# audio-visual/Audio_Visual_Deepfake_Detection

Measured on NVIDIA B200. Metric: videos/sec localization inference (fwd+decode+soft-NMS), higher is better.
Workload: dtype bf16

## Files before the change

audio_visual_deepfake_detection_b200/csrc/mlp_fused.cu:

```cuda
#include <cuda.h>
#include <stdlib.h>
#include <string.h>
#include "../../include/avdf.h"
#include "tc_ptx.cuh"

namespace avdf {
namespace mlpf {
using namespace tc;

constexpr int C = 256, HID = 1024, BM = 128, HC = 128, NCHUNK = HID / HC;
constexpr int UNIT = 128 * 64 * 2;
constexpr int RING = 5;
#ifndef AVDF_MLP_GELU_WARPS
#define AVDF_MLP_GELU_WARPS 8
#endif
constexpr int EPI_WARPS = 8;
constexpr int GELU_WARPS = AVDF_MLP_GELU_WARPS;
static_assert(GELU_WARPS == 8 || GELU_WARPS == 16, "GELU warps");
constexpr int GCOLS = HC / (GELU_WARPS / 4);
constexpr int THREADS = 128 + GELU_WARPS * 32;
constexpr int OFF_X = 0;
constexpr int OFF_H = OFF_X + 4 * UNIT;
constexpr int OFF_STG = OFF_H + 2 * UNIT;
constexpr int OFF_RING = OFF_STG + EPI_WARPS * 4096;
constexpr int OFF_VEC = OFF_RING + RING * UNIT;
constexpr int OFF_PART = OFF_VEC + (HID + 6 * C) * 4;
constexpr int OFF_BAR = OFF_PART + 2 * BM * 8;
constexpr int SMEM_BYTES = OFF_BAR + 512 + 1024;

struct Params {
  CUtensorMap x_map, w1_map, w2_map;
  CUtensorMap res_map, out_map;
  CUtensorMap att_map, wo_map, skip_map;
  const float* bo; const float* gamma_a; const float* ln2_w; const float* ln2_b;
  int y_store;
  void* out_h;
  const float* b1; const float* b2; const float* gamma; const unsigned char* row_mask;
  int rows, tiles;
  int oh_t, oh_pitch, oh_row0;
  unsigned idesc, idesc2;
  unsigned long long* dbg;
};
__device__ __forceinline__ unsigned long long gtime_ns() { unsigned long long t; asm volatile("mov.u64 %0, %globaltimer;" : "=l"(t)); return t; }
#define MLPF_TS(role, slot) do { if (p.dbg && blockIdx.x == 0 && it == 0 && (slot) < 96 && (threadIdx.x & 31) == 0) p.dbg[(role) * 96 + (slot)] = gtime_ns(); } while (0)

enum { B_XFULL = 0, B_XEMPTY, B_RFULL, B_REMPTY = B_RFULL + RING, B_A1FULL = B_REMPTY + RING, B_A1EMPTY = B_A1FULL + 2,
       B_HFULL = B_A1EMPTY + 2, B_HEMPTY, B_A2FULL, B_A2EMPTY, B_ATTFULL, B_ATTEMPTY, B_RES, B_RES2 = B_RES + 2 * EPI_WARPS,
       B_COUNT = B_RES2 + 2 * EPI_WARPS };
static_assert(B_COUNT * 8 + 8 <= 512, "barrier block");

template <bool F16, bool PROJ>
__global__ void __launch_bounds__(THREADS, 1) mlp_fused_kernel(const __grid_constant__ Params p) {
  extern __shared__ unsigned char smem_dyn[];
  unsigned char* smem = smem_dyn + ((1024u - (smem_u32(smem_dyn) & 1023u)) & 1023u);
  unsigned char* sx = smem + OFF_X;
  unsigned char* sh = smem + OFF_H;
  unsigned char* sstg = smem + OFF_STG;
  unsigned char* sring = smem + OFF_RING;
  float* s_b1 = reinterpret_cast<float*>(smem + OFF_VEC);
  float* s_b2 = s_b1 + HID;
  float* s_gam = s_b2 + C;
  float* s_bo = s_gam + C; float* s_gama = s_bo + C; float* s_l2w = s_gama + C; float* s_l2b = s_l2w + C;
  float2* s_part = reinterpret_cast<float2*>(smem + OFF_PART);
  uint64_t* bars = reinterpret_cast<uint64_t*>(smem + OFF_BAR);
  uint32_t* tmem_ptr_smem = reinterpret_cast<uint32_t*>(bars + B_COUNT);
  const uint32_t bar_base = smem_u32(bars);
  auto bar = [&](int i) { return bar_base + 8u * (uint32_t)i; };
  const int warp = threadIdx.x >> 5, lane = threadIdx.x & 31;
  const uint32_t rank = cluster_ctarank();
  const int unit0 = (int)(blockIdx.x >> 1), unit_step = (int)(gridDim.x >> 1), n_units = (p.tiles + 1) / 2;
  auto lbar = [&](int i) { return mapa_rank(bar(i), 0u); };
  auto chunk_of = [&](int j) { return j; };

  if (warp == 0 && lane == 0) {
    asm volatile("prefetch.tensormap [%0];" ::"l"(&p.x_map) : "memory");
    asm volatile("prefetch.tensormap [%0];" ::"l"(&p.w1_map) : "memory");
    asm volatile("prefetch.tensormap [%0];" ::"l"(&p.w2_map) : "memory");
    asm volatile("prefetch.tensormap [%0];" ::"l"(&p.res_map) : "memory");
    asm volatile("prefetch.tensormap [%0];" ::"l"(&p.out_map) : "memory");
    if (PROJ) {
      asm volatile("prefetch.tensormap [%0];" ::"l"(&p.att_map) : "memory");
      asm volatile("prefetch.tensormap [%0];" ::"l"(&p.wo_map) : "memory");
      asm volatile("prefetch.tensormap [%0];" ::"l"(&p.skip_map) : "memory");
    }
  }
  if (warp == 1 && lane == 0) {
    mbar_init(bar(B_XFULL), PROJ ? 2 * EPI_WARPS : 1); mbar_init(bar(B_XEMPTY), 1);
    mbar_init(bar(B_ATTFULL), 1); mbar_init(bar(B_ATTEMPTY), EPI_WARPS);
    for (int s = 0; s < RING; ++s) { mbar_init(bar(B_RFULL + s), 1); mbar_init(bar(B_REMPTY + s), 1); }
    for (int s = 0; s < 2; ++s) { mbar_init(bar(B_A1FULL + s), 1); mbar_init(bar(B_A1EMPTY + s), 2 * GELU_WARPS); }
    mbar_init(bar(B_HFULL), 2 * GELU_WARPS); mbar_init(bar(B_HEMPTY), 1);
    mbar_init(bar(B_A2FULL), 1); mbar_init(bar(B_A2EMPTY), 2 * EPI_WARPS);
    for (int s = 0; s < 4 * EPI_WARPS; ++s) mbar_init(bar(B_RES + s), 1);
    asm volatile("fence.mbarrier_init.release.cluster;" ::: "memory");
  }
  if (warp == 2) {
    asm volatile("tcgen05.alloc.cta_group::2.sync.aligned.shared::cta.b32 [%0], %1;" ::"r"(smem_u32(tmem_ptr_smem)), "r"(512u) : "memory");
    asm volatile("tcgen05.relinquish_alloc_permit.cta_group::2.sync.aligned;" ::: "memory");
  }
  if (warp >= 4) {
    for (int i = threadIdx.x - 128; i < HID; i += GELU_WARPS * 32) s_b1[i] = p.b1 ? __ldg(p.b1 + i) : 0.f;
    for (int i = threadIdx.x - 128; i < C; i += GELU_WARPS * 32) {
      s_b2[i] = p.b2 ? __ldg(p.b2 + i) : 0.f;
      s_gam[i] = p.gamma ? __ldg(p.gamma + i) : 1.f;
      if (PROJ) {
        s_bo[i] = p.bo ? __ldg(p.bo + i) : 0.f;
        s_gama[i] = p.gamma_a ? __ldg(p.gamma_a + i) : 1.f;
        s_l2w[i] = __ldg(p.ln2_w + i); s_l2b[i] = __ldg(p.ln2_b + i);
      }
    }
  }
  tcgen05_fence_before();
  cluster_sync_all();
  tcgen05_fence_after();
  const uint32_t tmem_base = *tmem_ptr_smem;
  const uint32_t tm_acc2 = tmem_base + 256u;
  pdl_trigger();
  pdl_wait();

  if (warp == 0) {
    const bool leader = elect_one();
    int stage = 0; uint32_t phase = 0; int it = 0;
    int nu = 0;
    auto begin_slot = [&]() -> uint32_t {
      mbar_wait(bar(B_REMPTY + stage), phase ^ 1);
      MLPF_TS(0, 1 + nu); ++nu;
      if (leader && rank == 0) mbar_arrive_expect_tx(bar(B_RFULL + stage), 2 * UNIT);
      return lbar(B_RFULL + stage);
    };
    auto end_slot = [&]() { __syncwarp(); if (++stage == RING) { stage = 0; phase ^= 1; } };
    auto load_w1 = [&](int chunk, int u) {
      const uint32_t fb = begin_slot();
      if (leader) {
        tma_load_2d_pair(smem_u32(sring + stage * UNIT), &p.w1_map, fb, (2 * u) * 64, chunk * HC + (int)rank * 64);
        tma_load_2d_pair(smem_u32(sring + stage * UNIT + UNIT / 2), &p.w1_map, fb, (2 * u + 1) * 64, chunk * HC + (int)rank * 64);
      }
      end_slot();
    };
    auto load_w2 = [&](int chunk, int sl) {
      const uint32_t fb = begin_slot();
      if (leader) tma_load_2d_pair(smem_u32(sring + stage * UNIT), &p.w2_map, fb, chunk * HC + sl * 64, (int)rank * 128);
      end_slot();
    };
    for (int unit = unit0; unit < n_units; unit += unit_step, ++it) {
      const int tile = 2 * unit + (int)rank;
      nu = 0;
      if (!PROJ) {
        mbar_wait(bar(B_XEMPTY), (uint32_t)(it & 1) ^ 1);
        MLPF_TS(0, 0);
        if (leader) {
          if (rank == 0) mbar_arrive_expect_tx(bar(B_XFULL), 8 * UNIT);
          const uint32_t xb = lbar(B_XFULL);
          for (int s = 0; s < 4; ++s) tma_load_2d_pair(smem_u32(sx + s * UNIT), &p.x_map, xb, s * 64, tile * BM);
        }
        __syncwarp();
      } else {
        mbar_wait(bar(B_ATTEMPTY), (uint32_t)(it & 1) ^ 1);
        MLPF_TS(0, 0);
        if (leader) {
          if (rank == 0) mbar_arrive_expect_tx(bar(B_ATTFULL), 8 * UNIT);
          const uint32_t ab = lbar(B_ATTFULL);
          for (int s = 0; s < 4; ++s) tma_load_2d_pair(smem_u32(sh + s * UNIT), &p.att_map, ab, s * 64, tile * BM);
        }
        __syncwarp();
        for (int sl = 0; sl < 4; ++sl) {
          const uint32_t fb = begin_slot();
          if (leader) tma_load_2d_pair(smem_u32(sring + stage * UNIT), &p.wo_map, fb, sl * 64, (int)rank * 128);
          end_slot();
        }
      }
      for (int u = 0; u < 2; ++u) load_w1(chunk_of(0), u);
      for (int j = 0; j < NCHUNK; ++j) {
        if (j + 1 < NCHUNK)
          for (int u = 0; u < 2; ++u) load_w1(chunk_of(j + 1), u);
        for (int sl = 0; sl < 2; ++sl) load_w2(chunk_of(j), sl);
      }
    }
  } else if (warp == 1 && rank == 0) {
    const bool leader = elect_one();
    int stage = 0; uint32_t phase = 0; int it = 0;
    uint32_t n_a1[2] = {0, 0}, n_h = 0, n_a2e = 0;
    auto g1 = [&](int j) {
      const int b = j & 1;
      mbar_wait(bar(B_A1EMPTY + b), (n_a1[b] & 1) ^ 1);
      tcgen05_fence_after();
      for (int u = 0; u < 2; ++u) {
        mbar_wait(bar(B_RFULL + stage), phase);
        tcgen05_fence_after();
        if (leader) {
#pragma unroll
          for (int ks = 0; ks < 2; ++ks) {
            const uint64_t da = make_sw128_desc(smem_u32(sx + (2 * u + ks) * UNIT));
            const uint64_t db = make_sw128_desc(smem_u32(sring + stage * UNIT + ks * (UNIT / 2)));
#pragma unroll
            for (int k = 0; k < 4; ++k)
              umma_bf16_pair(tmem_base + (uint32_t)(b * HC), da + (uint64_t)(2 * k), db + (uint64_t)(2 * k), p.idesc, (u > 0 || ks > 0 || k > 0) ? 1u : 0u);
          }
          umma_commit_pair(bar(B_REMPTY + stage));
          if (u == 1) umma_commit_pair(bar(B_A1FULL + b));
        }
        __syncwarp();
        if (++stage == RING) { stage = 0; phase ^= 1; }
      }
      ++n_a1[b];
    };
    for (int unit = unit0; unit < n_units; unit += unit_step, ++it) {
      if (PROJ) {
        mbar_wait(bar(B_A2EMPTY), (n_a2e & 1) ^ 1); ++n_a2e;
        mbar_wait(bar(B_ATTFULL), (uint32_t)(it & 1));
        tcgen05_fence_after();
        for (int sl = 0; sl < 4; ++sl) {
          mbar_wait(bar(B_RFULL + stage), phase);
          tcgen05_fence_after();
          if (leader) {
            const uint64_t da = make_sw128_desc(smem_u32(sh + sl * UNIT));
            const uint64_t db = make_sw128_desc(smem_u32(sring + stage * UNIT));
#pragma unroll
            for (int k = 0; k < 4; ++k)
              umma_bf16_pair(tm_acc2, da + (uint64_t)(2 * k), db + (uint64_t)(2 * k), p.idesc2, (sl > 0 || k > 0) ? 1u : 0u);
            umma_commit_pair(bar(B_REMPTY + stage));
            if (sl == 3) umma_commit_pair(bar(B_A2FULL));
          }
          __syncwarp();
          if (++stage == RING) { stage = 0; phase ^= 1; }
        }
      }
      mbar_wait(bar(B_XFULL), (uint32_t)(it & 1));
      tcgen05_fence_after();
      MLPF_TS(1, 0);
      g1(0);
      MLPF_TS(1, 1);
      for (int j = 0; j < NCHUNK; ++j) {
        if (j + 1 < NCHUNK) g1(j + 1);
        MLPF_TS(1, 2 + 4 * j);
        if (j == NCHUNK - 2 && leader) umma_commit_pair(bar(B_XEMPTY));
        if (j == 0) { mbar_wait(bar(B_A2EMPTY), (n_a2e & 1) ^ 1); ++n_a2e; tcgen05_fence_after(); }
        mbar_wait(bar(B_HFULL), n_h & 1);
        tcgen05_fence_after();
        MLPF_TS(1, 3 + 4 * j);
        for (int sl = 0; sl < 2; ++sl) {
          mbar_wait(bar(B_RFULL + stage), phase);
          tcgen05_fence_after();
          if (leader) {
            const uint64_t da = make_sw128_desc(smem_u32(sh + sl * UNIT));
            const uint64_t db = make_sw128_desc(smem_u32(sring + stage * UNIT));
#pragma unroll
            for (int k = 0; k < 4; ++k)
              umma_bf16_pair(tm_acc2, da + (uint64_t)(2 * k), db + (uint64_t)(2 * k), p.idesc2, (PROJ || j > 0 || sl > 0 || k > 0) ? 1u : 0u);
            umma_commit_pair(bar(B_REMPTY + stage));
          }
          __syncwarp();
          if (++stage == RING) { stage = 0; phase ^= 1; }
        }
        if (leader) {
          umma_commit_pair(bar(B_HEMPTY));
          if (j == NCHUNK - 1) umma_commit_pair(bar(B_A2FULL));
        }
        __syncwarp();
        ++n_h;
        MLPF_TS(1, 4 + 4 * j);
      }
    }
  } else if (warp >= 4) {
    const int wi = warp - 4;
    const int q = warp & 3;
    const int cg = wi >> 2;
    const int g = cg & 1;
    const bool fin = wi < EPI_WARPS;
    const int r = q * 32 + lane;
    const int sw7 = lane & 7;
    unsigned char* tA = sstg + (wi & 7) * 4096;
    unsigned char* tB = sh + (wi & 7) * 4096;
    const uint32_t res_bar[2] = {bar(B_RES + 2 * (wi & 7)), bar(B_RES + 2 * (wi & 7) + 1)};
    uint32_t res_phase[2] = {0, 0};
    const uint32_t a1empty_bar[2] = {lbar(B_A1EMPTY), lbar(B_A1EMPTY + 1)};
    const uint32_t hfull_bar = lbar(B_HFULL), a2empty_bar = lbar(B_A2EMPTY);
    uint32_t n_a1[2] = {0, 0}, n_h = 0, n_a2f = 0;
    const uint32_t xfull_bar = lbar(B_XFULL);
    int it = 0;
    for (int unit = unit0; unit < n_units; unit += unit_step, ++it) {
      const int tile = 2 * unit + (int)rank;
      const int row = tile * BM + r;
      float mk = 1.f;
      if (p.row_mask) mk = (row < p.rows && __ldg(p.row_mask + row)) ? 1.f : 0.f;
      const int wrow = tile * BM + q * 32;
      const int col0 = g * 128;
      auto fetch_residual = [&](int ch) {
        mbar_arrive_expect_tx(res_bar[ch & 1], 4096);
        tma_load_2d(smem_u32((ch & 1) ? tB : tA), &p.res_map, res_bar[ch & 1], col0 + ch * 32, wrow);
      };
      if (!PROJ && fin && lane == 0) fetch_residual(0);
      if (PROJ) {
        unsigned char* tX[4] = {sx + wi * 8192, sx + wi * 8192 + 4096, tA, tB};
        const uint32_t sk_bar[4] = {res_bar[0], res_bar[1], bar(B_RES2 + 2 * wi), bar(B_RES2 + 2 * wi + 1)};
        auto fetch_skip = [&](int ch) {
          mbar_arrive_expect_tx(sk_bar[ch], 4096);
          tma_load_2d(smem_u32(tX[ch]), &p.skip_map, sk_bar[ch], col0 + ch * 32, wrow);
        };
        mbar_wait(bar(B_XEMPTY), (uint32_t)(it & 1) ^ 1);
        if (lane == 0) { fetch_skip(0); fetch_skip(1); }
        if (wi == 0 && lane == 0) MLPF_TS(2, 42);
        mbar_wait(bar(B_A2FULL), n_a2f & 1); ++n_a2f;
        tcgen05_fence_after();
        if (wi == 0 && lane == 0) MLPF_TS(2, 43);
        if (lane == 0) { fetch_skip(2); fetch_skip(3); }
        const uint32_t taddr2 = tm_acc2 + ((uint32_t)(q * 32) << 16) + (uint32_t)col0;
        float s = 0.f, ss = 0.f;
        uint32_t vr[32];
        tmem_ld32_issue(taddr2, vr);
#pragma unroll 1
        for (int ch = 0; ch < 4; ++ch) {
          tmem_ld_wait();
          float x[32];
#pragma unroll
          for (int i = 0; i < 32; ++i) x[i] = __uint_as_float(vr[i]);
          if (ch + 1 < 4) tmem_ld32_issue(taddr2 + (ch + 1) * 32, vr);
          unsigned char* tb = tX[ch];
          if (ch < 2) { mbar_wait(sk_bar[ch], res_phase[ch]); res_phase[ch] ^= 1; }
          else mbar_wait(sk_bar[ch], (uint32_t)(it & 1));
          const float4* b4 = reinterpret_cast<const float4*>(s_bo + col0 + ch * 32);
          const float4* g4 = reinterpret_cast<const float4*>(s_gama + col0 + ch * 32);
          uint32_t yb[32];
#pragma unroll
          for (int jj = 0; jj < 8; ++jj) {
            float4* slot = reinterpret_cast<float4*>(tb + lane * 128 + ((jj ^ sw7) << 4));
            const float4 rv = *slot;
            const float4 bb = b4[jj], gg = g4[jj];
            const float4 y = make_float4(fmaf(gg.x, (x[4 * jj] + bb.x) * mk, rv.x * mk), fmaf(gg.y, (x[4 * jj + 1] + bb.y) * mk, rv.y * mk),
                                         fmaf(gg.z, (x[4 * jj + 2] + bb.z) * mk, rv.z * mk), fmaf(gg.w, (x[4 * jj + 3] + bb.w) * mk, rv.w * mk));
            *slot = y;
            s += (y.x + y.y) + (y.z + y.w);
            ss = fmaf(y.x, y.x, ss); ss = fmaf(y.y, y.y, ss); ss = fmaf(y.z, y.z, ss); ss = fmaf(y.w, y.w, ss);
            yb[4 * jj] = __float_as_uint(y.x); yb[4 * jj + 1] = __float_as_uint(y.y); yb[4 * jj + 2] = __float_as_uint(y.z); yb[4 * jj + 3] = __float_as_uint(y.w);
          }
          tmem_st32(taddr2 + ch * 32, yb);
          if (p.y_store) {
            fence_async_smem();
            __syncwarp();
            if (lane == 0) {
              tma_store_2d(&p.res_map, smem_u32(tb), col0 + ch * 32, wrow);
              tma_store_commit();
            }
          } else {
            __syncwarp();
          }
        }
        if (wi == 0 && lane == 0) MLPF_TS(2, 44);
        s_part[g * BM + r] = make_float2(s, ss);
        asm volatile("bar.sync %0, 64;" ::"r"(2 + q) : "memory");
        const float2 pa = s_part[r], pb = s_part[BM + r];
        const float mean = (pa.x + pb.x) * (1.f / C);
        const float rstd = rsqrtf(fmaxf((pa.y + pb.y) * (1.f / C) - mean * mean, 0.f) + 1e-5f);
        tmem_st_wait();
        if (p.y_store && lane == 0) tma_store_wait_read();
        asm volatile("bar.sync 1, %0;" ::"n"(EPI_WARPS * 32) : "memory");
        const f32x2 nmean2 = pk2(-mean), rstd2 = pk2(rstd);
#pragma unroll 1
        for (int ch = 0; ch < 4; ++ch) {
          uint32_t vy[32];
          tmem_ld32_issue(taddr2 + ch * 32, vy);
          tmem_ld_wait();
          if (ch == 3) {
            tcgen05_fence_before();
            __syncwarp();
            if (lane == 0) mbar_arrive_cluster(a2empty_bar);
          }
          const int c0 = col0 + ch * 32;
          unsigned char* xrow = sx + (c0 >> 6) * UNIT + r * 128;
          const int slot0 = (c0 & 63) >> 3;
          const float4* w4 = reinterpret_cast<const float4*>(s_l2w + c0);
          const float4* l4 = reinterpret_cast<const float4*>(s_l2b + c0);
#pragma unroll
          for (int jj = 0; jj < 4; ++jj) {
            f32x2 y[4];
#pragma unroll
            for (int u = 0; u < 2; ++u) {
              const float4 ww = w4[2 * jj + u], ll = l4[2 * jj + u];
              y[2 * u] = fma2(mul2(add2(pk2(__uint_as_float(vy[8 * jj + 4 * u]), __uint_as_float(vy[8 * jj + 4 * u + 1])), nmean2), rstd2), pk2(ww.x, ww.y), pk2(ll.x, ll.y));
              y[2 * u + 1] = fma2(mul2(add2(pk2(__uint_as_float(vy[8 * jj + 4 * u + 2]), __uint_as_float(vy[8 * jj + 4 * u + 3])), nmean2), rstd2), pk2(ww.z, ww.w), pk2(ll.z, ll.w));
            }
            uint4 uo;
            float f0, f1;
            if (F16) {
              upk2(y[0], f0, f1); uo.x = pack_f16x2(f0, f1); upk2(y[1], f0, f1); uo.y = pack_f16x2(f0, f1);
              upk2(y[2], f0, f1); uo.z = pack_f16x2(f0, f1); upk2(y[3], f0, f1); uo.w = pack_f16x2(f0, f1);
            } else {
              upk2(y[0], f0, f1); uo.x = pack_bf16x2(f0, f1); upk2(y[1], f0, f1); uo.y = pack_bf16x2(f0, f1);
              upk2(y[2], f0, f1); uo.z = pack_bf16x2(f0, f1); upk2(y[3], f0, f1); uo.w = pack_bf16x2(f0, f1);
            }
            *reinterpret_cast<uint4*>(xrow + (((slot0 + jj) ^ sw7) << 4)) = uo;
          }
        }
        fence_async_smem();
        __syncwarp();
        if (wi == 0 && lane == 0) MLPF_TS(2, 45);
        if (lane == 0) mbar_arrive_cluster(xfull_bar);
      }
      for (int j = 0; j < NCHUNK; ++j) {
        const int b = j & 1;
        mbar_wait(bar(B_A1FULL + b), n_a1[b] & 1);
        ++n_a1[b];
        tcgen05_fence_after();
        if (wi == 0 && lane == 0) MLPF_TS(2, 4 * j);
        const uint32_t taddr = tmem_base + ((uint32_t)(q * 32) << 16) + (uint32_t)(b * HC + cg * GCOLS);
        uint32_t va[GCOLS];
        tmem_ld32_issue(taddr, *reinterpret_cast<uint32_t(*)[32]>(va));
        if (GCOLS == 64) tmem_ld32_issue(taddr + 32, *reinterpret_cast<uint32_t(*)[32]>(va + GCOLS - 32));
        tmem_ld_wait();
        tcgen05_fence_before();
        __syncwarp();
        if (lane == 0) mbar_arrive_cluster(a1empty_bar[b]);
        unsigned char* hrow = sh + ((cg * GCOLS) >> 6) * UNIT + r * 128;
        const int slot0 = ((cg * GCOLS) & 63) >> 3;
        const float* bias = s_b1 + chunk_of(j) * HC + cg * GCOLS;
        uint4 hv[GCOLS / 8];
        const float4* b4 = reinterpret_cast<const float4*>(bias);
#pragma unroll
        for (int jj = 0; jj < GCOLS / 8; ++jj) {
          f32x2 y[4];
#pragma unroll
          for (int u = 0; u < 2; ++u) {
            const float4 bb = b4[2 * jj + u];
            y[2 * u] = gelu_poly2(add2(pk2(__uint_as_float(va[8 * jj + 4 * u]), __uint_as_float(va[8 * jj + 4 * u + 1])), pk2(bb.x, bb.y)));
            y[2 * u + 1] = gelu_poly2(add2(pk2(__uint_as_float(va[8 * jj + 4 * u + 2]), __uint_as_float(va[8 * jj + 4 * u + 3])), pk2(bb.z, bb.w)));
          }
          uint4 uo;
          float f0, f1;
          if (F16) {
            upk2(y[0], f0, f1); uo.x = pack_f16x2(f0, f1); upk2(y[1], f0, f1); uo.y = pack_f16x2(f0, f1);
            upk2(y[2], f0, f1); uo.z = pack_f16x2(f0, f1); upk2(y[3], f0, f1); uo.w = pack_f16x2(f0, f1);
          } else {
            upk2(y[0], f0, f1); uo.x = pack_bf16x2(f0, f1); upk2(y[1], f0, f1); uo.y = pack_bf16x2(f0, f1);
            upk2(y[2], f0, f1); uo.z = pack_bf16x2(f0, f1); upk2(y[3], f0, f1); uo.w = pack_bf16x2(f0, f1);
          }
          hv[jj] = uo;
        }
        if (wi == 0 && lane == 0) MLPF_TS(2, 4 * j + 1);
        mbar_wait(bar(B_HEMPTY), (n_h & 1) ^ 1);
        ++n_h;
        if (wi == 0 && lane == 0) MLPF_TS(2, 4 * j + 2);
#pragma unroll
        for (int c = 0; c < GCOLS / 8; ++c) *reinterpret_cast<uint4*>(hrow + (((slot0 + c) ^ sw7) << 4)) = hv[c];
        fence_async_smem();
        __syncwarp();
        if (lane == 0) mbar_arrive_cluster(hfull_bar);
        if (wi == 0 && lane == 0) MLPF_TS(2, 4 * j + 3);
      }
      if (fin) {
      mbar_wait(bar(B_A2FULL), n_a2f & 1); ++n_a2f;
      tcgen05_fence_after();
      if (wi == 0 && lane == 0) MLPF_TS(2, 40);
      if (!PROJ && lane == 0) fetch_residual(1);
      const uint32_t taddr2 = tm_acc2 + ((uint32_t)(q * 32) << 16) + (uint32_t)col0;
      unsigned short* outh_base = p.out_h ? reinterpret_cast<unsigned short*>(p.out_h) + col0 + lane : nullptr;
      int my_dr = wrow + lane;
      if (p.out_h && p.oh_t) my_dr = (my_dr / p.oh_t) * p.oh_pitch + p.oh_row0 + (my_dr % p.oh_t);
      const int nrow = min(32, p.rows - wrow);
      uint32_t vr[32];
      tmem_ld32_issue(taddr2, vr);
#pragma unroll 1
      for (int ch = 0; ch < 4; ++ch) {
        tmem_ld_wait();
        float x[32];
#pragma unroll
        for (int i = 0; i < 32; ++i) x[i] = __uint_as_float(vr[i]);
        if (ch + 1 < 4) {
          tmem_ld32_issue(taddr2 + (ch + 1) * 32, vr);
        } else {
          tcgen05_fence_before();
          __syncwarp();
          if (lane == 0) mbar_arrive_cluster(a2empty_bar);
        }
        unsigned char* tb = (ch & 1) ? tB : tA;
        const float4* b4 = reinterpret_cast<const float4*>(s_b2 + col0 + ch * 32);
        if (PROJ) {
          if (ch >= 2) {
            if (lane == 0) asm volatile("cp.async.bulk.wait_group.read 1;" ::: "memory");
            __syncwarp();
          }
#pragma unroll
          for (int jj = 0; jj < 8; ++jj) {
            const float4 bb = b4[jj];
            *reinterpret_cast<float4*>(tb + lane * 128 + ((jj ^ sw7) << 4)) =
                make_float4((x[4 * jj] + bb.x) * mk, (x[4 * jj + 1] + bb.y) * mk, (x[4 * jj + 2] + bb.z) * mk, (x[4 * jj + 3] + bb.w) * mk);
          }
        } else {
        if (ch >= 1 && ch + 1 < 4 && lane == 0) {
          tma_store_wait_read();
          fetch_residual(ch + 1);
        }
        mbar_wait(res_bar[ch & 1], res_phase[ch & 1]);
        res_phase[ch & 1] ^= 1;
        const float4* g4 = reinterpret_cast<const float4*>(s_gam + col0 + ch * 32);
#pragma unroll
        for (int jj = 0; jj < 8; ++jj) {
          float4* slot = reinterpret_cast<float4*>(tb + lane * 128 + ((jj ^ sw7) << 4));
          const float4 rv = *slot;
          const float4 bb = b4[jj], gg = g4[jj];
          *slot = make_float4(fmaf(rv.x, mk, gg.x * ((x[4 * jj] + bb.x) * mk)), fmaf(rv.y, mk, gg.y * ((x[4 * jj + 1] + bb.y) * mk)),
                              fmaf(rv.z, mk, gg.z * ((x[4 * jj + 2] + bb.z) * mk)), fmaf(rv.w, mk, gg.w * ((x[4 * jj + 3] + bb.w) * mk)));
        }
        }
        fence_async_smem();
        __syncwarp();
        if (lane == 0) {
          tma_store_2d(&p.out_map, smem_u32(tb), col0 + ch * 32, wrow);
          tma_store_commit();
        }
        if (outh_base != nullptr) {
#pragma unroll 8
          for (int rr = 0; rr < 32; ++rr) {
            const float o = *reinterpret_cast<const float*>(tb + rr * 128 + ((((lane >> 2) ^ (rr & 7)) << 4) | ((lane & 3) << 2)));
            const int dr = __shfl_sync(0xffffffffu, my_dr, rr);
            unsigned short hb;
            if (F16) { const __half hh = __float2half_rn(o); hb = *reinterpret_cast<const unsigned short*>(&hh); }
            else { const __nv_bfloat16 hh = __float2bfloat16_rn(o); hb = *reinterpret_cast<const unsigned short*>(&hh); }
            if (rr < nrow) outh_base[(size_t)dr * C + ch * 32] = hb;
          }
          __syncwarp();
        }
      }
      if (wi == 0 && lane == 0) MLPF_TS(2, 41);
      if (lane == 0) {
        tma_store_wait_read();
        if (PROJ) mbar_arrive(bar(B_ATTEMPTY));
      }
      }
      asm volatile("bar.sync 1, %0;" ::"n"(GELU_WARPS * 32) : "memory");
    }
    if (fin && lane == 0) asm volatile("cp.async.bulk.wait_group 0;" ::: "memory");
  }
  tcgen05_fence_before();
  cluster_sync_all();
  if (warp == 2) {
    tcgen05_fence_after();
    asm volatile("tcgen05.dealloc.cta_group::2.sync.aligned.b32 %0, %1;" ::"r"(tmem_base), "r"(512u) : "memory");
  }
}

}
}

using namespace avdf;

static unsigned long long* g_mlpf_dbg = nullptr;
extern "C" __attribute__((visibility("default"))) int avdf_debug_mlp_timeline(unsigned long long* dev_buf) {
  g_mlpf_dbg = dev_buf;
  return 0;
}

extern "C" int avdf_mlp_fused(const avdf_mlp_fused_args* a, void* stream) {
  using namespace avdf::mlpf;
  AVDF_CHECK_ARG(a != nullptr, "args is null");
  AVDF_CHECK_ARG(a->channels == C && a->hidden == HID, "avdf_mlp_fused supports channels = 256, hidden = 1024");
  AVDF_CHECK_ARG(a->dtype == AVDF_DTYPE_F16 || a->dtype == AVDF_DTYPE_BF16, "dtype must be a 16-bit type");
  AVDF_CHECK_ARG(a->rows >= 0, "rows must be >= 0");
  const bool proj = a->att != nullptr;
  AVDF_CHECK_ARG(a->w1 && a->w2 && a->out, "null pointer");
  if (proj) {
    AVDF_CHECK_ARG(a->w_o && a->ln2_w && a->ln2_b && a->skip, "block tail: w_o, ln2_w, ln2_b and skip are required");
    AVDF_CHECK_ARG(a->gamma == nullptr, "block tail: fold the MLP's scale into w2 / b2 (gamma must be NULL)");
    AVDF_CHECK_ARG(((reinterpret_cast<uintptr_t>(a->att) | reinterpret_cast<uintptr_t>(a->w_o) | reinterpret_cast<uintptr_t>(a->skip) |
                     reinterpret_cast<uintptr_t>(a->y)) & 15) == 0, "pointers must be 16-byte aligned");
    AVDF_CHECK_ARG(GELU_WARPS == EPI_WARPS, "block tail needs the eight-warp build");
  } else {
    AVDF_CHECK_ARG(a->x && a->residual, "null pointer");
  }
  AVDF_CHECK_ARG(((reinterpret_cast<uintptr_t>(proj ? a->att : a->x) | reinterpret_cast<uintptr_t>(a->w1) | reinterpret_cast<uintptr_t>(a->w2) |
                   reinterpret_cast<uintptr_t>(proj ? nullptr : a->residual) | reinterpret_cast<uintptr_t>(a->out)) & 15) == 0, "pointers must be 16-byte aligned");
  if (a->rows == 0) return AVDF_OK;
  tc::EncodeFn encode = tc::get_encode();
  if (!encode) { set_error("avdf_mlp_fused: cuTensorMapEncodeTiled not available from the driver"); return AVDF_ERR_CUDA; }
  const bool f16 = a->dtype == AVDF_DTYPE_F16;
  const CUtensorMapDataType dt = f16 ? CU_TENSOR_MAP_DATA_TYPE_FLOAT16 : CU_TENSOR_MAP_DATA_TYPE_BFLOAT16;
  static thread_local Params p;
  memset(&p, 0, sizeof(p));
  auto enc2 = [&](CUtensorMap* m, CUtensorMapDataType t, int es, const void* base, long long cols, long long rows_, int bc, int br,
                  const char* what) -> int {
    cuuint64_t dims[2] = {(cuuint64_t)cols, (cuuint64_t)rows_};
    cuuint64_t strides[1] = {(cuuint64_t)cols * es};
    cuuint32_t box[2] = {(cuuint32_t)bc, (cuuint32_t)br};
    cuuint32_t estr[2] = {1, 1};
    CUresult r = encode(m, t, 2, const_cast<void*>(base), dims, strides, box, estr, CU_TENSOR_MAP_INTERLEAVE_NONE,
                        CU_TENSOR_MAP_SWIZZLE_128B, CU_TENSOR_MAP_L2_PROMOTION_L2_256B, CU_TENSOR_MAP_FLOAT_OOB_FILL_NONE);
    if (r != CUDA_SUCCESS) { set_error("avdf_mlp_fused: cuTensorMapEncodeTiled(%s) failed with %d", what, (int)r); return AVDF_ERR_CUDA; }
    return AVDF_OK;
  };
  int rc;
  if (!proj && (rc = enc2(&p.x_map, dt, 2, a->x, C, a->rows, 64, 128, "x"))) return rc;
  if (proj) {
    if ((rc = enc2(&p.att_map, dt, 2, a->att, C, a->rows, 64, 128, "att"))) return rc;
    if ((rc = enc2(&p.wo_map, dt, 2, a->w_o, C, C, 64, 128, "w_o"))) return rc;
    if ((rc = enc2(&p.skip_map, CU_TENSOR_MAP_DATA_TYPE_FLOAT32, 4, a->skip, C, a->rows, 32, 32, "skip"))) return rc;
    p.bo = a->b_o; p.gamma_a = a->gamma_attn; p.ln2_w = a->ln2_w; p.ln2_b = a->ln2_b;
  }
  if ((rc = enc2(&p.w1_map, dt, 2, a->w1, C, HID, 64, 64, "w1"))) return rc;
  if ((rc = enc2(&p.w2_map, dt, 2, a->w2, HID, C, 64, 128, "w2"))) return rc;
  p.y_store = (proj && a->y) ? 1 : 0;
  if ((!proj || a->y) && (rc = enc2(&p.res_map, CU_TENSOR_MAP_DATA_TYPE_FLOAT32, 4, proj ? a->y : a->residual, C, a->rows, 32, 32, "residual"))) return rc;
  if ((rc = enc2(&p.out_map, CU_TENSOR_MAP_DATA_TYPE_FLOAT32, 4, a->out, C, a->rows, 32, 32, "out"))) return rc;
  p.out_h = a->out_h;
  p.oh_t = a->out_h_t; p.oh_pitch = a->out_h_pitch; p.oh_row0 = a->out_h_row0;
  AVDF_CHECK_ARG(a->out_h_t >= 0 && (a->out_h_t == 0 || (a->rows % a->out_h_t == 0 && a->out_h_pitch >= a->out_h_t + a->out_h_row0)),
                 "out_h_t must divide rows and fit the destination pitch");
  AVDF_CHECK_ARG(!a->out_h || (reinterpret_cast<uintptr_t>(a->out_h) & 15) == 0, "out_h must be 16-byte aligned");
  p.b1 = a->b1; p.b2 = a->b2; p.gamma = a->gamma; p.row_mask = a->row_mask;
  p.rows = a->rows; p.tiles = (a->rows + BM - 1) / BM;
  p.dbg = g_mlpf_dbg;
  const unsigned fmt = f16 ? 0u : 1u;
  const unsigned m_field = (unsigned)((2 * BM) >> 4) << 24;
  p.idesc = (1u << 4) | (fmt << 7) | (fmt << 10) | ((unsigned)(128 >> 3) << 17) | m_field;
  p.idesc2 = (1u << 4) | (fmt << 7) | (fmt << 10) | ((unsigned)(256 >> 3) << 17) | m_field;
  const int sms = device_sm_count();
  AVDF_SMEM_ATTR_ONCE((mlp_fused_kernel<true, false>), SMEM_BYTES);
  AVDF_SMEM_ATTR_ONCE((mlp_fused_kernel<false, false>), SMEM_BYTES);
  AVDF_SMEM_ATTR_ONCE((mlp_fused_kernel<true, true>), SMEM_BYTES);
  AVDF_SMEM_ATTR_ONCE((mlp_fused_kernel<false, true>), SMEM_BYTES);
  cudaStream_t st = reinterpret_cast<cudaStream_t>(stream);
  const int units = (p.tiles + 1) / 2, max_pairs = sms / 2;
  const int grid = 2 * (units < max_pairs ? units : max_pairs);
  cudaError_t lerr;
  if (proj) lerr = f16 ? launch_pdl_cluster(mlp_fused_kernel<true, true>, grid, THREADS, SMEM_BYTES, st, 2, p)
                       : launch_pdl_cluster(mlp_fused_kernel<false, true>, grid, THREADS, SMEM_BYTES, st, 2, p);
  else lerr = f16 ? launch_pdl_cluster(mlp_fused_kernel<true, false>, grid, THREADS, SMEM_BYTES, st, 2, p)
                  : launch_pdl_cluster(mlp_fused_kernel<false, false>, grid, THREADS, SMEM_BYTES, st, 2, p);
  if (lerr != cudaSuccess) { set_error("mlp_fused_kernel: launch failed: %s", cudaGetErrorString(lerr)); return AVDF_ERR_CUDA; }
  return check_launch("mlp_fused_kernel");
}
```

Before: 21580.

## Load attention tile into X buffer and drop ATTEMPTY barrier in proj MLP

In the PROJ variant, the attention tile now goes into the sx buffer and uses the XEMPTY barrier, the same path as the non-proj case. The separate ATTEMPTY barrier and the epilogue's extra wait on XEMPTY are removed. The skip staging buffers are reordered so the first two chunks use the tA/tB scratch instead of sx, which avoids conflicts with the next attention tile. The proj launch grid is also resized so each CTA pair handles a balanced number of tiles. The intent is to let the next tile's attention load overlap sooner with the epilogue, at the risk of subtle buffer-reuse hazards.

Measured after the change: 21570 (median of 6 runs). No clear change (-0.0%).

```diff
diff --git a/audio_visual_deepfake_detection_b200/csrc/mlp_fused.cu b/audio_visual_deepfake_detection_b200/csrc/mlp_fused.cu
--- a/audio_visual_deepfake_detection_b200/csrc/mlp_fused.cu
+++ b/audio_visual_deepfake_detection_b200/csrc/mlp_fused.cu
@@ -42,10 +42,10 @@
   unsigned long long* dbg;
 };
 __device__ __forceinline__ unsigned long long gtime_ns() { unsigned long long t; asm volatile("mov.u64 %0, %globaltimer;" : "=l"(t)); return t; }
-#define MLPF_TS(role, slot) do { if (p.dbg && blockIdx.x == 0 && it == 0 && (slot) < 96 && (threadIdx.x & 31) == 0) p.dbg[(role) * 96 + (slot)] = gtime_ns(); } while (0)
+#define MLPF_TS(role, slot) do { if (p.dbg && blockIdx.x == 0 && it < 2 && (slot) < 96 && (threadIdx.x & 31) == 0) p.dbg[(it * 3 + (role)) * 96 + (slot)] = gtime_ns(); } while (0)
 
 enum { B_XFULL = 0, B_XEMPTY, B_RFULL, B_REMPTY = B_RFULL + RING, B_A1FULL = B_REMPTY + RING, B_A1EMPTY = B_A1FULL + 2,
-       B_HFULL = B_A1EMPTY + 2, B_HEMPTY, B_A2FULL, B_A2EMPTY, B_ATTFULL, B_ATTEMPTY, B_RES, B_RES2 = B_RES + 2 * EPI_WARPS,
+       B_HFULL = B_A1EMPTY + 2, B_HEMPTY, B_A2FULL, B_A2EMPTY, B_ATTFULL, B_RES, B_RES2 = B_RES + 2 * EPI_WARPS,
        B_COUNT = B_RES2 + 2 * EPI_WARPS };
 static_assert(B_COUNT * 8 + 8 <= 512, "barrier block");
 
@@ -86,7 +86,7 @@
   }
   if (warp == 1 && lane == 0) {
     mbar_init(bar(B_XFULL), PROJ ? 2 * EPI_WARPS : 1); mbar_init(bar(B_XEMPTY), 1);
-    mbar_init(bar(B_ATTFULL), 1); mbar_init(bar(B_ATTEMPTY), EPI_WARPS);
+    mbar_init(bar(B_ATTFULL), 1);
     for (int s = 0; s < RING; ++s) { mbar_init(bar(B_RFULL + s), 1); mbar_init(bar(B_REMPTY + s), 1); }
     for (int s = 0; s < 2; ++s) { mbar_init(bar(B_A1FULL + s), 1); mbar_init(bar(B_A1EMPTY + s), 2 * GELU_WARPS); }
     mbar_init(bar(B_HFULL), 2 * GELU_WARPS); mbar_init(bar(B_HEMPTY), 1);
@@ -145,24 +145,15 @@
     for (int unit = unit0; unit < n_units; unit += unit_step, ++it) {
       const int tile = 2 * unit + (int)rank;
       nu = 0;
-      if (!PROJ) {
-        mbar_wait(bar(B_XEMPTY), (uint32_t)(it & 1) ^ 1);
-        MLPF_TS(0, 0);
-        if (leader) {
-          if (rank == 0) mbar_arrive_expect_tx(bar(B_XFULL), 8 * UNIT);
-          const uint32_t xb = lbar(B_XFULL);
-          for (int s = 0; s < 4; ++s) tma_load_2d_pair(smem_u32(sx + s * UNIT), &p.x_map, xb, s * 64, tile * BM);
-        }
-        __syncwarp();
-      } else {
-        mbar_wait(bar(B_ATTEMPTY), (uint32_t)(it & 1) ^ 1);
-        MLPF_TS(0, 0);
-        if (leader) {
-          if (rank == 0) mbar_arrive_expect_tx(bar(B_ATTFULL), 8 * UNIT);
-          const uint32_t ab = lbar(B_ATTFULL);
-          for (int s = 0; s < 4; ++s) tma_load_2d_pair(smem_u32(sh + s * UNIT), &p.att_map, ab, s * 64, tile * BM);
-        }
-        __syncwarp();
+      mbar_wait(bar(B_XEMPTY), (uint32_t)(it & 1) ^ 1);
+      MLPF_TS(0, 0);
+      if (leader) {
+        if (rank == 0) mbar_arrive_expect_tx(bar(PROJ ? B_ATTFULL : B_XFULL), 8 * UNIT);
+        const uint32_t xb = lbar(PROJ ? B_ATTFULL : B_XFULL);
+        for (int s = 0; s < 4; ++s) tma_load_2d_pair(smem_u32(sx + s * UNIT), PROJ ? &p.att_map : &p.x_map, xb, s * 64, tile * BM);
+      }
+      __syncwarp();
+      if (PROJ) {
         for (int sl = 0; sl < 4; ++sl) {
           const uint32_t fb = begin_slot();
           if (leader) tma_load_2d_pair(smem_u32(sring + stage * UNIT), &p.wo_map, fb, sl * 64, (int)rank * 128);
@@ -213,7 +204,7 @@
           mbar_wait(bar(B_RFULL + stage), phase);
           tcgen05_fence_after();
           if (leader) {
-            const uint64_t da = make_sw128_desc(smem_u32(sh + sl * UNIT));
+            const uint64_t da = make_sw128_desc(smem_u32(sx + sl * UNIT));
             const uint64_t db = make_sw128_desc(smem_u32(sring + stage * UNIT));
 #pragma unroll
             for (int k = 0; k < 4; ++k)
@@ -291,13 +282,12 @@
       };
       if (!PROJ && fin && lane == 0) fetch_residual(0);
       if (PROJ) {
-        unsigned char* tX[4] = {sx + wi * 8192, sx + wi * 8192 + 4096, tA, tB};
+        unsigned char* tX[4] = {tA, tB, sx + wi * 8192, sx + wi * 8192 + 4096};
         const uint32_t sk_bar[4] = {res_bar[0], res_bar[1], bar(B_RES2 + 2 * wi), bar(B_RES2 + 2 * wi + 1)};
         auto fetch_skip = [&](int ch) {
           mbar_arrive_expect_tx(sk_bar[ch], 4096);
           tma_load_2d(smem_u32(tX[ch]), &p.skip_map, sk_bar[ch], col0 + ch * 32, wrow);
         };
-        mbar_wait(bar(B_XEMPTY), (uint32_t)(it & 1) ^ 1);
         if (lane == 0) { fetch_skip(0); fetch_skip(1); }
         if (wi == 0 && lane == 0) MLPF_TS(2, 42);
         mbar_wait(bar(B_A2FULL), n_a2f & 1); ++n_a2f;
@@ -521,10 +511,7 @@
         }
       }
       if (wi == 0 && lane == 0) MLPF_TS(2, 41);
-      if (lane == 0) {
-        tma_store_wait_read();
-        if (PROJ) mbar_arrive(bar(B_ATTEMPTY));
-      }
+      if (lane == 0) tma_store_wait_read();
       }
       asm volatile("bar.sync 1, %0;" ::"n"(GELU_WARPS * 32) : "memory");
     }
@@ -618,7 +605,9 @@
   AVDF_SMEM_ATTR_ONCE((mlp_fused_kernel<false, true>), SMEM_BYTES);
   cudaStream_t st = reinterpret_cast<cudaStream_t>(stream);
   const int units = (p.tiles + 1) / 2, max_pairs = sms / 2;
-  const int grid = 2 * (units < max_pairs ? units : max_pairs);
+  const int per_pair = proj ? (units + max_pairs - 1) / max_pairs : 1;
+  const int pairs = (units + per_pair - 1) / per_pair;
+  const int grid = 2 * (pairs < max_pairs ? pairs : max_pairs);
   cudaError_t lerr;
   if (proj) lerr = f16 ? launch_pdl_cluster(mlp_fused_kernel<true, true>, grid, THREADS, SMEM_BYTES, st, 2, p)
                        : launch_pdl_cluster(mlp_fused_kernel<false, true>, grid, THREADS, SMEM_BYTES, st, 2, p);
```
